# georgeretsi/smirk

Measured on AMD Instinct MI355X. Metric: faces/sec (encode+FLAME+render+generate) @224x224, higher is better.
Workload: dtype f32 results; encoder + generator convs as split-fp16 x3 MFMA with f32 accumulate (fp32-class error), FLAME / raster f32; 1 GPU; BASELINE config 4: full inference incl. SmirkGenerator re-synthesis, 1024-frame batch sharded over the GPUs; global_batch=1024, micro_batch=1024, image=224x224, parallelism=dp1, rccl_ranks_seen=1, collective=none (1 GPU), hw_queues=4

## Files before the change

smirk_amd/csrc/mbconv_image.hip:

```cpp
#include <stdio.h>

#include "common.h"

typedef _Float16 half8 __attribute__((ext_vector_type(8)));

struct MBIArgs {
    const char* x;
    const char* wexp;
    const float *s1, *b1;
    const float* wdw;
    const float *s2, *b2;
    const char* wproj;
    const float *s3, *b3;
    char* out;
    int B, H, W, Cin, mid, Cout, residual, ipw, rows, gsz, nb;
    int off_es, off_wp, off_wc, off_gmap;
    int tile, tiles_x, tiles_y, gpitch;
    int rowsE, nbE, off_gmapE;
};

__device__ __forceinline__ void mbi_barrier() {
    asm volatile("s_waitcnt lgkmcnt(0)" ::: "memory");
    __builtin_amdgcn_s_barrier();
    asm volatile("" ::: "memory");
}

__device__ __forceinline__ int mbi_es(int gi, int c) { return gi * 32 + ((((c >> 2) ^ (gi >> 1)) & 7) << 2) + (c & 3); }

template <int KS, int NT, bool TILE = false, bool PADK = false>
__global__ __launch_bounds__(512, 2) void mbconv_image_kernel(MBIArgs a) {
    extern __shared__ __attribute__((aligned(16))) char mbi_smem[];
    SmirkRangeAccS rng;
    const int strideX = KS * 64 + 16;
    char* Xs = mbi_smem;
    float* Es = (float*)(mbi_smem + a.off_es);
    char* Wp = mbi_smem + a.off_wp;
    float* Wc = (float*)(mbi_smem + a.off_wc);
    short* gmap = (short*)(mbi_smem + a.off_gmap);
    short* gmapE = TILE ? (short*)(mbi_smem + a.off_gmapE) : gmap;
    const int tid = threadIdx.x, lane = tid & 63, wave = tid >> 6, fr = lane & 31, hb = lane >> 5;
    const int ntile = a.tiles_x * a.tiles_y;
    const int tb = TILE ? (int)blockIdx.x / ntile : 0, tt = TILE ? (int)blockIdx.x - tb * ntile : 0;
    const int ty = tt / a.tiles_x, tx = tt - ty * a.tiles_x;
    const int b0 = TILE ? tb : blockIdx.x * a.ipw;
    const int nimg = min(a.ipw, a.B - b0), HW = a.H * a.W, vrows = TILE ? 196 : nimg * HW;
    const int nchunks = (a.mid + 31) / 32;
    const size_t xrow = (size_t)a.Cin * 4;
    const half8 hz = {0, 0, 0, 0, 0, 0, 0, 0};
    const int swave = __builtin_amdgcn_readfirstlane(wave);
    const bool active = swave < a.nb;
    const bool activeE = TILE ? swave < a.nbE : active;
    const int wpbuf = a.Cout * 144;

    half8 we[KS][2];
    float s1v = 0.f, b1v = 0.f;
    auto load_we = [&](int c) {
        int frw = fr;
        asm volatile("" : "+v"(frw));
        const int ch = 32 * c + frw;
        const bool v = ch < a.mid;
        const int chc = min(ch, a.mid - 1);
        const char* wbase = a.wexp;
        asm volatile("" : "+s"(wbase));
        const char* wrow = wbase + (unsigned)chc * (unsigned)(a.Cin * 4);
#pragma unroll
        for (int s = 0; s < KS; ++s) {
            const int g = 2 * s + hb;
            if constexpr (PADK) {
                const int gc = min(g, a.Cin / 8 - 1);
                const half8 t0 = *(const half8*)(wrow + gc * 32), t1h = *(const half8*)(wrow + gc * 32 + 16);
                we[s][0] = g * 8 < a.Cin ? t0 : hz;
                we[s][1] = g * 8 < a.Cin ? t1h : hz;
            } else {
                we[s][0] = *(const half8*)(wrow + g * 32);
                we[s][1] = *(const half8*)(wrow + g * 32 + 16);
            }
        }
        const float t1 = a.s1[chc], t2 = a.b1[chc];
        s1v = v ? t1 : 0.f;
        b1v = v ? t2 : 0.f;
    };
    f32x4 wpv[2];
    float wcv = 0.f;
    auto fetch_stage = [&](int c) {
        int t0 = tid;
        asm volatile("" : "+v"(t0));
#pragma unroll
        for (int u = 0; u < 2; ++u) {
            const int idx = t0 + 512 * u, row = idx >> 3, piece = idx & 7, kg = 4 * c + (piece >> 1);
            const bool ok = row < a.Cout && kg * 8 < a.mid;
            const int rc = min(row, a.Cout - 1), kc = min(kg, a.mid / 8 - 1);
            const f32x4 t = *(const f32x4*)(a.wproj + ((size_t)rc * a.mid + kc * 8) * 4 + (piece & 1) * 16);
            const f32x4 z = {0.f, 0.f, 0.f, 0.f};
            wpv[u] = ok ? t : z;
        }
        {
            const int k = min(t0 >> 5, 10), ch = 32 * c + (t0 & 31), chc = min(ch, a.mid - 1);
            const float* src = k < 9 ? a.wdw + (size_t)k * a.mid : (k == 9 ? a.s2 : a.b2);
            const float t = src[chc];
            wcv = ch < a.mid ? t : 0.f;
        }
    };
    auto store_stage = [&](int c) {
        char* dst = Wp + (c & 1) * wpbuf;
        int t0 = tid;
        asm volatile("" : "+v"(t0));
#pragma unroll
        for (int u = 0; u < 2; ++u) {
            const int idx = t0 + 512 * u, row = idx >> 3, piece = idx & 7;
            if (row < a.Cout) *(f32x4*)(dst + row * 144 + piece * 16) = wpv[u];
        }
        if (t0 < 352) Wc[(c & 1) * 352 + t0] = wcv;
    };

    {
        const int P = a.Cin / 4;
        const char* xb = a.x + (size_t)b0 * HW * xrow;
        const int rowsE = TILE ? 256 : a.rows, total = rowsE * P, vtotal = vrows * P;
        for (int base = 0; base < total; base += 512 * 4) {
            f32x4 xv[4];
#pragma unroll
            for (int u = 0; u < 4; ++u) {
                const int idx = base + 512 * u + tid;
                const f32x4 z = {0.f, 0.f, 0.f, 0.f};
                if (TILE) {
                    const int c = min(idx / P, 255), pc = idx - (idx / P) * P;
                    const int gy = ty * 14 - 1 + (c >> 4), gx = tx * 14 - 1 + (c & 15);
                    const bool ok = idx < total && gy >= 0 && gy < a.H && gx >= 0 && gx < a.W;
                    const int yc = min(max(gy, 0), a.H - 1), xc = min(max(gx, 0), a.W - 1);
                    const f32x4 t = *(const f32x4*)(xb + ((size_t)yc * a.W + xc) * xrow + pc * 16);
                    xv[u] = ok ? t : z;
                } else {
                    const f32x4 t = *(const f32x4*)(xb + (size_t)min(idx, vtotal - 1) * 16);
                    xv[u] = idx < vtotal ? t : z;
                }
            }
#pragma unroll
            for (int u = 0; u < 4; ++u) {
                const int idx = base + 512 * u + tid, row = idx / P, pc = idx - row * P;
                if (idx < total) *(f32x4*)(Xs + row * strideX + pc * 16) = xv[u];
            }
        }
        if (PADK && KS * 4 > P) {
            const int PP = KS * 4 - P;
            for (int idx = tid; idx < rowsE * PP; idx += 512) {
                const int row = idx / PP, pc = P + idx - row * PP;
                *(f32x4*)(Xs + row * strideX + pc * 16) = f32x4{0.f, 0.f, 0.f, 0.f};
            }
        }
        for (int idx = tid; idx < a.gsz * 8; idx += 512) ((f32x4*)Es)[idx] = f32x4{0.f, 0.f, 0.f, 0.f};
        for (int r = tid; r < a.nb * 32; r += 512) {
            int g = -1;
            if (r < vrows) {
                if (TILE) {
                    const int iy = r / 14, ix = r - iy * 14;
                    g = (iy + 1) * 16 + ix + 1;
                } else {
                    const int im = r / HW, rem = r - im * HW, y = rem / a.W, xx = rem - y * a.W;
                    g = (im * (a.H + 2) + y + 1) * (a.W + 2) + xx + 1;
                }
            }
            gmap[r] = (short)g;
        }
        if (TILE)
            for (int r = tid; r < a.nbE * 32; r += 512) {
                const int gy = ty * 14 - 1 + (r >> 4), gx = tx * 14 - 1 + (r & 15);
                const bool ok = r < 256 && gy >= 0 && gy < a.H && gx >= 0 && gx < a.W;
                gmapE[r] = (short)(ok ? r : ~min(r, 255));
            }
    }
    mbi_barrier();

    f32x16 pacc[NT][2];
#pragma unroll
    for (int q = 0; q < NT; ++q)
#pragma unroll
        for (int h = 0; h < 2; ++h)
#pragma unroll
            for (int r = 0; r < 16; ++r) pacc[q][h][r] = 0.f;
    const int myrow = min(wave * 32 + fr, (TILE ? 256 : a.rows) - 1);
    const int mygi = active ? (int)gmap[min(wave * 32 + fr, a.nb * 32 - 1)] : -1;

    auto expand = [&]() {
        if (!activeE) return;
        f32x16 e0, e1;
#pragma unroll
        for (int r = 0; r < 16; ++r) { e0[r] = 0.f; e1[r] = 0.f; }
        const char* arow = Xs + myrow * strideX;
#pragma unroll
        for (int s = 0; s < KS; ++s) {
            const int g = 2 * s + hb;
            const half8 ah = *(const half8*)(arow + g * 32), al = *(const half8*)(arow + g * 32 + 16);
            e0 = __builtin_amdgcn_mfma_f32_32x32x16_f16(ah, we[s][0], e0, 0, 0, 0);
            e1 = __builtin_amdgcn_mfma_f32_32x32x16_f16(ah, we[s][1], e1, 0, 0, 0);
            e1 = __builtin_amdgcn_mfma_f32_32x32x16_f16(al, we[s][0], e1, 0, 0, 0);
            if ((s & 1) || NT == 4) __builtin_amdgcn_sched_barrier(0);
        }
        int rbase = wave * 32 + 4 * hb;
        asm volatile("" : "+v"(rbase));
#pragma unroll
        for (int r = 0; r < 16; ++r) {
            const int gm = gmapE[rbase + (r & 3) + 8 * (r >> 2)];
            const float v = fmaxf((e0[r] + e1[r] * (1.0f / 2048.0f)) * s1v + b1v, 0.f);
            Es[mbi_es(gm >= 0 ? gm : ~gm, fr)] = gm >= 0 ? v : 0.f;
        }
    };


    for (int c = -1; c < nchunks; ++c) {
        const bool more = c + 1 < nchunks;
        if (more) fetch_stage(c + 1);
        half8 dh[2] = {hz, hz}, dl[2] = {hz, hz};
        if (c >= 0 && active && mygi >= 0) {
            const float* wc = Wc + (c & 1) * 352;
#pragma unroll
            for (int s = 0; s < 2; ++s) {
                const int c8 = 8 * (2 * s + hb);
                int gc = mygi;
                asm volatile("" : "+v"(gc));
                float acc[8] = {0.f, 0.f, 0.f, 0.f, 0.f, 0.f, 0.f, 0.f};
#pragma unroll
                for (int ky = 0; ky < 3; ++ky)
#pragma unroll
                    for (int kx = 0; kx < 3; ++kx) {
                        const int gi = gc + (ky - 1) * a.gpitch + (kx - 1);
                        const f32x4 v0 = *(const f32x4*)(Es + mbi_es(gi, c8)), v1 = *(const f32x4*)(Es + mbi_es(gi, c8 + 4));
                        const f32x4 w0 = *(const f32x4*)(wc + (ky * 3 + kx) * 32 + c8), w1 = *(const f32x4*)(wc + (ky * 3 + kx) * 32 + c8 + 4);
#pragma unroll
                        for (int q = 0; q < 4; ++q) { acc[q] = fmaf(v0[q], w0[q], acc[q]); acc[4 + q] = fmaf(v1[q], w1[q], acc[4 + q]); }
                        if (kx == 2 || NT == 4) __builtin_amdgcn_sched_barrier(0);
                    }
                const f32x4 sa = *(const f32x4*)(wc + 9 * 32 + c8), sb = *(const f32x4*)(wc + 9 * 32 + c8 + 4);
                const f32x4 ba = *(const f32x4*)(wc + 10 * 32 + c8), bb = *(const f32x4*)(wc + 10 * 32 + c8 + 4);
#pragma unroll
                for (int q = 0; q < 8; ++q) {
                    const float v = fmaxf(acc[q] * (q < 4 ? sa[q & 3] : sb[q & 3]) + (q < 4 ? ba[q & 3] : bb[q & 3]), 0.f);
                    _Float16 h, l;
                    smirk_split1(v, h, l);
                    dh[s][q] = h; dl[s][q] = l;
                }
            }
        }
        if (more) store_stage(c + 1);
        mbi_barrier();
        if (more) load_we(c + 1);
        if (c >= 0 && active) {
            const char* wp = Wp + (c & 1) * wpbuf;
            int frq = fr;
            asm volatile("" : "+v"(frq));
#pragma unroll
            for (int q = 0; q < NT; ++q) {
                const int co = min(q * 32 + frq, a.Cout - 1);
                const char* brow = wp + co * 144;
#pragma unroll
                for (int s = 0; s < 2; ++s) {
                    const int g = 2 * s + hb;
                    const half8 bhh = *(const half8*)(brow + g * 32), bll = *(const half8*)(brow + g * 32 + 16);
                    pacc[q][0] = __builtin_amdgcn_mfma_f32_32x32x16_f16(dh[s], bhh, pacc[q][0], 0, 0, 0);
                    pacc[q][1] = __builtin_amdgcn_mfma_f32_32x32x16_f16(dh[s], bll, pacc[q][1], 0, 0, 0);
                    pacc[q][1] = __builtin_amdgcn_mfma_f32_32x32x16_f16(dl[s], bhh, pacc[q][1], 0, 0, 0);
                }
                __builtin_amdgcn_sched_barrier(0);
            }
        }
        if (more) expand();
        mbi_barrier();
    }

    if (active) {
        const int lane = __builtin_amdgcn_mbcnt_hi(~0u, __builtin_amdgcn_mbcnt_lo(~0u, 0u)), wave = swave, fr = lane & 31;
        float* tb = Es + wave * (32 * 36);
        char* ob = a.out + (size_t)b0 * HW * a.Cout * 4;
#pragma unroll
        for (int q = 0; q < NT; ++q) {
            if (q * 32 < a.Cout) {
                const int co = q * 32 + fr;
                const float s3 = co < a.Cout ? a.s3[co] : 0.f, b3 = co < a.Cout ? a.b3[co] : 0.f;
#pragma unroll
                for (int r = 0; r < 16; ++r) tb[mfma32_row(r, lane) * 36 + fr] = (pacc[q][0][r] + pacc[q][1][r] * (1.0f / 2048.0f)) * s3 + b3;
                asm volatile("s_waitcnt lgkmcnt(0)" ::: "memory");
#pragma unroll
                for (int it = 0; it < 2; ++it) {
                    const int item = it * 64 + lane, row = item >> 2, g8 = q * 4 + (item & 3);
                    const int r = wave * 32 + row;
                    if (r < vrows && g8 * 8 < a.Cout) {
                        const int iy = r / 14, ix = r - iy * 14;
                        const int xrow_i = TILE ? (iy + 1) * 16 + ix + 1 : r;
                        const size_t opix = TILE ? (size_t)(ty * 14 + iy) * a.W + tx * 14 + ix : (size_t)r;
                        float v[8];
                        *(f32x4*)v = *(const f32x4*)(tb + row * 36 + (item & 3) * 8);
                        *(f32x4*)(v + 4) = *(const f32x4*)(tb + row * 36 + (item & 3) * 8 + 4);
                        if (a.residual) {
                            const char* xr = Xs + xrow_i * strideX + g8 * 32;
                            const half8 hi = *(const half8*)xr, lo = *(const half8*)(xr + 16);
#pragma unroll
                            for (int k = 0; k < 8; ++k) v[k] += (float)hi[k] + (float)lo[k] * (1.0f / 2048.0f);
                        }
                        half8 hi, lo;
                        rng.see8(v);
#pragma unroll
                        for (int k = 0; k < 8; ++k) {
                            _Float16 h, l;
                            smirk_split1(v[k], h, l);
                            hi[k] = h; lo[k] = l;
                        }
                        char* o = ob + (opix * a.Cout + g8 * 8) * 4;
                        *(half8*)o = hi;
                        *(half8*)(o + 16) = lo;
                    }
                }
                asm volatile("s_waitcnt lgkmcnt(0)" ::: "memory");
            }
        }
    }
    rng.commit();
}

struct MbiPlan { int ipw, rows, gsz, nb, off_es, off_wp, off_wc, off_gmap, tile, tiles_x, tiles_y, gpitch, rowsE, nbE, off_gmapE; size_t lds; };
static bool mbi_plan(int H, int W, int Cin, int mid, int Cout, MbiPlan& p) {
    if (H <= 0 || W <= 0 || Cin % 8 || mid % 8 || Cout % 8 || Cin < 16 || Cin > 112 || Cout > 128 || mid <= 0 || Cout <= 0) return false;
    const int KS = (Cin + 15) / 16;
    p.tile = H * W > 224 ? 1 : 0;
    if (p.tile) {
        if (H % 14 || W % 14) return false;
        p.tiles_x = W / 14; p.tiles_y = H / 14; p.gpitch = 16;
        p.ipw = 1; p.rows = 196; p.gsz = 256; p.nb = 7; p.rowsE = 256; p.nbE = 8;
    } else {
        p.tiles_x = p.tiles_y = 1; p.gpitch = W + 2;
        p.ipw = 224 / (H * W);
        if (p.ipw > 8) p.ipw = 8;
        p.rows = p.ipw * H * W;
        p.gsz = p.ipw * (H + 2) * (W + 2);
        p.nb = (p.rows + 31) / 32;
        p.rowsE = p.rows; p.nbE = p.nb;
    }
    if (p.nb > 7 || p.gsz * 128 < p.nb * 32 * 36 * 4) return false;
    size_t o = (size_t)p.rowsE * (KS * 64 + 16);
    o = (o + 15) / 16 * 16; p.off_es = (int)o; o += (size_t)p.gsz * 128;
    p.off_wp = (int)o; o += (size_t)2 * Cout * 144;
    p.off_wc = (int)o; o += 2 * 352 * 4;
    p.off_gmap = (int)o; o += (size_t)p.nb * 32 * 2;
    p.off_gmapE = p.off_gmap;
    if (p.tile) { p.off_gmapE = (int)o; o += (size_t)p.nbE * 32 * 2; }
    p.lds = (o + 15) / 16 * 16;
    return p.lds <= 160 * 1024;
}

static bool mbi_has_variant(int ks, int nt) {
    return (ks == 5 && (nt == 2 || nt == 3 || nt == 4)) || (ks == 6 && (nt == 3 || nt == 4)) || (ks == 7 && (nt == 3 || nt == 4)) ||
           (ks == 4 && (nt == 2 || nt == 3)) || (ks == 2 && nt == 1) || (ks == 3 && nt == 2);
}

extern "C" int smirk_mbconv_image_supported(int H, int W, int Cin, int mid, int Cout, int stride) {
    MbiPlan p;
    if (stride != 1 || !mbi_plan(H, W, Cin, mid, Cout, p)) return 0;
    const int ks = (Cin + 15) / 16, nt = (Cout + 31) / 32;
    if (!mbi_has_variant(ks, nt)) return 0;
    const bool small = (ks == 2 && nt == 1) || (ks == 3 && nt == 2);
    return (small || (!p.tile && Cin % 16 == 0)) ? 1 : 0;
}

template <int KS, int NT, bool TILE = false, bool PADK = false>
static int mbi_launch(const MBIArgs& a, unsigned grid, size_t lds, hipStream_t st) {
    if (const int rc = smirk_raise_dynamic_lds((const void*)mbconv_image_kernel<KS, NT, TILE, PADK>, 160 * 1024)) return rc;
    if (g_smirk_prof_on) {
        char nm[64];
        if (TILE || PADK) snprintf(nm, sizeof(nm), "mbconv_image_kernel<%d,%d,%s,%s>", KS, NT, TILE ? "true" : "false", PADK ? "true" : "false");
        else snprintf(nm, sizeof(nm), "mbconv_image_kernel<%d,%d>", KS, NT);
        const double px = (double)a.B * a.H * a.W;
        smirk_prof_next_mbconv(nm, px, px, a.Cin, a.mid, a.Cout, true, a.residual != 0);
    }
    SMIRK_LAUNCH((mbconv_image_kernel<KS, NT, TILE, PADK>), dim3(grid), dim3(512), lds, st, a);
    return smirk_launch_status();
}

extern "C" int smirk_mbconv_image_split16(const void* x, const void* wexp, const float* s1, const float* b1, const float* wdw, const float* s2,
                                          const float* b2, const void* wproj, const float* s3, const float* b3, int residual, void* out, int B,
                                          int H, int W, int Cin, int mid, int Cout, void* stream) {
    if (!x || !wexp || !s1 || !b1 || !wdw || !s2 || !b2 || !wproj || !s3 || !b3 || !out || B <= 0) return SMIRK_ERR_BAD_ARG;
    if (residual && Cin != Cout) return SMIRK_ERR_BAD_ARG;
    MbiPlan p;
    if (!mbi_plan(H, W, Cin, mid, Cout, p) || !smirk_mbconv_image_supported(H, W, Cin, mid, Cout, 1)) return SMIRK_ERR_UNSUPPORTED;
    MBIArgs a;
    a.x = (const char*)x; a.wexp = (const char*)wexp; a.s1 = s1; a.b1 = b1; a.wdw = wdw; a.s2 = s2; a.b2 = b2; a.wproj = (const char*)wproj;
    a.s3 = s3; a.b3 = b3; a.out = (char*)out; a.B = B; a.H = H; a.W = W; a.Cin = Cin; a.mid = mid; a.Cout = Cout; a.residual = residual;
    a.ipw = p.ipw; a.rows = p.rows; a.gsz = p.gsz; a.nb = p.nb; a.off_es = p.off_es; a.off_wp = p.off_wp; a.off_wc = p.off_wc; a.off_gmap = p.off_gmap;
    a.tile = p.tile; a.tiles_x = p.tiles_x; a.tiles_y = p.tiles_y; a.gpitch = p.gpitch; a.rowsE = p.rowsE; a.nbE = p.nbE; a.off_gmapE = p.off_gmapE;
    const unsigned grid = p.tile ? (unsigned)B * p.tiles_x * p.tiles_y : (unsigned)((B + p.ipw - 1) / p.ipw);
    hipStream_t st = (hipStream_t)stream;
    const int ks = (Cin + 15) / 16, nt = (Cout + 31) / 32;
#define MBI_CASE(K, N) if (ks == K && nt == N) return mbi_launch<K, N>(a, grid, p.lds, st)
    MBI_CASE(5, 3); MBI_CASE(5, 4); MBI_CASE(6, 3); MBI_CASE(7, 4);
    MBI_CASE(4, 2); MBI_CASE(4, 3); MBI_CASE(5, 2); MBI_CASE(6, 4); MBI_CASE(7, 3);
    if (ks == 2 && nt == 1) return p.tile ? mbi_launch<2, 1, true, true>(a, grid, p.lds, st) : mbi_launch<2, 1, false, true>(a, grid, p.lds, st);
    if (ks == 3 && nt == 2) return p.tile ? mbi_launch<3, 2, true, true>(a, grid, p.lds, st) : mbi_launch<3, 2, false, true>(a, grid, p.lds, st);
#undef MBI_CASE
    return SMIRK_ERR_UNSUPPORTED;
}
```

Before: 11390 faces/sec.

## Replace tiled MBConv path with per-wave 2x14 band kernel using 256 threads

The large-image (tiled) path of the fused MBConv kernel is rewritten. Each wave now processes its own 2-row by 14-column output band. Input activations and expand weights are held in registers, and the expanded tile lives in a small per-wave LDS buffer, so the kernel no longer stages a 16x16 haloed tile across 512 threads. Depthwise weights are staged in chunks shared by the four waves. The smaller LDS footprint and 256-thread blocks are meant to raise occupancy and drop the redundant halo expansion of 256 rows per 196 outputs. The trade-off is recomputing the expand for overlapping halo rows across adjacent bands (4 input rows per 2 output rows) and more global weight reloads per chunk.

```diff
diff --git a/smirk_amd/csrc/mbconv_image.hip b/smirk_amd/csrc/mbconv_image.hip
--- a/smirk_amd/csrc/mbconv_image.hip
+++ b/smirk_amd/csrc/mbconv_image.hip
@@ -15,9 +15,11 @@
     char* out;
     int B, H, W, Cin, mid, Cout, residual, ipw, rows, gsz, nb;
     int off_es, off_wp, off_wc, off_gmap;
-    int tile, tiles_x, tiles_y, gpitch;
-    int rowsE, nbE, off_gmapE;
+    int gpitch;
+    int tile, tiles_x, tiles_y, nbands;
 };
+
+extern __shared__ __attribute__((aligned(16))) char mbi_smem[];
 
 __device__ __forceinline__ void mbi_barrier() {
     asm volatile("s_waitcnt lgkmcnt(0)" ::: "memory");
@@ -27,9 +29,8 @@
 
 __device__ __forceinline__ int mbi_es(int gi, int c) { return gi * 32 + ((((c >> 2) ^ (gi >> 1)) & 7) << 2) + (c & 3); }
 
-template <int KS, int NT, bool TILE = false, bool PADK = false>
-__global__ __launch_bounds__(512, 2) void mbconv_image_kernel(MBIArgs a) {
-    extern __shared__ __attribute__((aligned(16))) char mbi_smem[];
+template <int KS, int NT, bool PADK>
+__device__ __forceinline__ void mbi_whole_body(const MBIArgs& a) {
     SmirkRangeAccS rng;
     const int strideX = KS * 64 + 16;
     char* Xs = mbi_smem;
@@ -37,19 +38,14 @@
     char* Wp = mbi_smem + a.off_wp;
     float* Wc = (float*)(mbi_smem + a.off_wc);
     short* gmap = (short*)(mbi_smem + a.off_gmap);
-    short* gmapE = TILE ? (short*)(mbi_smem + a.off_gmapE) : gmap;
     const int tid = threadIdx.x, lane = tid & 63, wave = tid >> 6, fr = lane & 31, hb = lane >> 5;
-    const int ntile = a.tiles_x * a.tiles_y;
-    const int tb = TILE ? (int)blockIdx.x / ntile : 0, tt = TILE ? (int)blockIdx.x - tb * ntile : 0;
-    const int ty = tt / a.tiles_x, tx = tt - ty * a.tiles_x;
-    const int b0 = TILE ? tb : blockIdx.x * a.ipw;
-    const int nimg = min(a.ipw, a.B - b0), HW = a.H * a.W, vrows = TILE ? 196 : nimg * HW;
+    const int b0 = blockIdx.x * a.ipw;
+    const int nimg = min(a.ipw, a.B - b0), HW = a.H * a.W, vrows = nimg * HW;
     const int nchunks = (a.mid + 31) / 32;
     const size_t xrow = (size_t)a.Cin * 4;
     const half8 hz = {0, 0, 0, 0, 0, 0, 0, 0};
     const int swave = __builtin_amdgcn_readfirstlane(wave);
     const bool active = swave < a.nb;
-    const bool activeE = TILE ? swave < a.nbE : active;
     const int wpbuf = a.Cout * 144;
 
     half8 we[KS][2];
@@ -116,24 +112,15 @@
     {
         const int P = a.Cin / 4;
         const char* xb = a.x + (size_t)b0 * HW * xrow;
-        const int rowsE = TILE ? 256 : a.rows, total = rowsE * P, vtotal = vrows * P;
+        const int total = a.rows * P, vtotal = vrows * P;
         for (int base = 0; base < total; base += 512 * 4) {
             f32x4 xv[4];
 #pragma unroll
             for (int u = 0; u < 4; ++u) {
                 const int idx = base + 512 * u + tid;
                 const f32x4 z = {0.f, 0.f, 0.f, 0.f};
-                if (TILE) {
-                    const int c = min(idx / P, 255), pc = idx - (idx / P) * P;
-                    const int gy = ty * 14 - 1 + (c >> 4), gx = tx * 14 - 1 + (c & 15);
-                    const bool ok = idx < total && gy >= 0 && gy < a.H && gx >= 0 && gx < a.W;
-                    const int yc = min(max(gy, 0), a.H - 1), xc = min(max(gx, 0), a.W - 1);
-                    const f32x4 t = *(const f32x4*)(xb + ((size_t)yc * a.W + xc) * xrow + pc * 16);
-                    xv[u] = ok ? t : z;
-                } else {
-                    const f32x4 t = *(const f32x4*)(xb + (size_t)min(idx, vtotal - 1) * 16);
-                    xv[u] = idx < vtotal ? t : z;
-                }
+                const f32x4 t = *(const f32x4*)(xb + (size_t)min(idx, vtotal - 1) * 16);
+                xv[u] = idx < vtotal ? t : z;
             }
 #pragma unroll
             for (int u = 0; u < 4; ++u) {
@@ -143,7 +130,7 @@
         }
         if (PADK && KS * 4 > P) {
             const int PP = KS * 4 - P;
-            for (int idx = tid; idx < rowsE * PP; idx += 512) {
+            for (int idx = tid; idx < a.rows * PP; idx += 512) {
                 const int row = idx / PP, pc = P + idx - row * PP;
                 *(f32x4*)(Xs + row * strideX + pc * 16) = f32x4{0.f, 0.f, 0.f, 0.f};
             }
@@ -152,22 +139,11 @@
         for (int r = tid; r < a.nb * 32; r += 512) {
             int g = -1;
             if (r < vrows) {
-                if (TILE) {
-                    const int iy = r / 14, ix = r - iy * 14;
-                    g = (iy + 1) * 16 + ix + 1;
-                } else {
-                    const int im = r / HW, rem = r - im * HW, y = rem / a.W, xx = rem - y * a.W;
-                    g = (im * (a.H + 2) + y + 1) * (a.W + 2) + xx + 1;
-                }
+                const int im = r / HW, rem = r - im * HW, y = rem / a.W, xx = rem - y * a.W;
+                g = (im * (a.H + 2) + y + 1) * (a.W + 2) + xx + 1;
             }
             gmap[r] = (short)g;
         }
-        if (TILE)
-            for (int r = tid; r < a.nbE * 32; r += 512) {
-                const int gy = ty * 14 - 1 + (r >> 4), gx = tx * 14 - 1 + (r & 15);
-                const bool ok = r < 256 && gy >= 0 && gy < a.H && gx >= 0 && gx < a.W;
-                gmapE[r] = (short)(ok ? r : ~min(r, 255));
-            }
     }
     mbi_barrier();
 
@@ -178,11 +154,11 @@
         for (int h = 0; h < 2; ++h)
 #pragma unroll
             for (int r = 0; r < 16; ++r) pacc[q][h][r] = 0.f;
-    const int myrow = min(wave * 32 + fr, (TILE ? 256 : a.rows) - 1);
+    const int myrow = min(wave * 32 + fr, a.rows - 1);
     const int mygi = active ? (int)gmap[min(wave * 32 + fr, a.nb * 32 - 1)] : -1;
 
     auto expand = [&]() {
-        if (!activeE) return;
+        if (!active) return;
         f32x16 e0, e1;
 #pragma unroll
         for (int r = 0; r < 16; ++r) { e0[r] = 0.f; e1[r] = 0.f; }
@@ -200,7 +176,7 @@
         asm volatile("" : "+v"(rbase));
 #pragma unroll
         for (int r = 0; r < 16; ++r) {
-            const int gm = gmapE[rbase + (r & 3) + 8 * (r >> 2)];
+            const int gm = gmap[rbase + (r & 3) + 8 * (r >> 2)];
             const float v = fmaxf((e0[r] + e1[r] * (1.0f / 2048.0f)) * s1v + b1v, 0.f);
             Es[mbi_es(gm >= 0 ? gm : ~gm, fr)] = gm >= 0 ? v : 0.f;
         }
@@ -284,15 +260,298 @@
                     const int item = it * 64 + lane, row = item >> 2, g8 = q * 4 + (item & 3);
                     const int r = wave * 32 + row;
                     if (r < vrows && g8 * 8 < a.Cout) {
-                        const int iy = r / 14, ix = r - iy * 14;
-                        const int xrow_i = TILE ? (iy + 1) * 16 + ix + 1 : r;
-                        const size_t opix = TILE ? (size_t)(ty * 14 + iy) * a.W + tx * 14 + ix : (size_t)r;
                         float v[8];
                         *(f32x4*)v = *(const f32x4*)(tb + row * 36 + (item & 3) * 8);
                         *(f32x4*)(v + 4) = *(const f32x4*)(tb + row * 36 + (item & 3) * 8 + 4);
                         if (a.residual) {
-                            const char* xr = Xs + xrow_i * strideX + g8 * 32;
+                            const char* xr = Xs + r * strideX + g8 * 32;
                             const half8 hi = *(const half8*)xr, lo = *(const half8*)(xr + 16);
+#pragma unroll
+                            for (int k = 0; k < 8; ++k) v[k] += (float)hi[k] + (float)lo[k] * (1.0f / 2048.0f);
+                        }
+                        half8 hi, lo;
+                        rng.see8(v);
+#pragma unroll
+                        for (int k = 0; k < 8; ++k) {
+                            _Float16 h, l;
+                            smirk_split1(v[k], h, l);
+                            hi[k] = h; lo[k] = l;
+                        }
+                        char* o = ob + ((size_t)r * a.Cout + g8 * 8) * 4;
+                        *(half8*)o = hi;
+                        *(half8*)(o + 16) = lo;
+                    }
+                }
+                asm volatile("s_waitcnt lgkmcnt(0)" ::: "memory");
+            }
+        }
+    }
+    rng.commit();
+}
+
+#define MBB_EB 8192
+#define MBB_STAGE 34
+
+__device__ __forceinline__ void mbb_out_px(int m, int& oy, int& ox) {
+    const int k = m >> 2;
+    oy = (0x96 >> k) & 1;
+    ox = (k >> 1) * 4 + (m & 3);
+}
+
+__device__ __forceinline__ void mbb_fence() { asm volatile("s_waitcnt lgkmcnt(0)" ::: "memory"); }
+
+template <int KS, int NT>
+__device__ __forceinline__ void mbi_band_body(const MBIArgs& a) {
+    SmirkRangeAccS rng;
+    const int tid = threadIdx.x, lane = tid & 63, fr = lane & 31, hb = lane >> 5;
+    const int wave = __builtin_amdgcn_readfirstlane(tid >> 6);
+    float* Wt = (float*)(mbi_smem + 4 * MBB_EB);
+    const int band = (int)blockIdx.x * 4 + wave;
+    const bool has = band < a.nbands;
+    int bid = min(band, a.nbands - 1);
+    const int bx = bid % a.tiles_x; bid /= a.tiles_x;
+    const int by = bid % a.tiles_y;
+    const int b = bid / a.tiles_y;
+    const int oy0 = by * 2, ox0 = bx * 14;
+    const bool interior = oy0 > 0 && oy0 + 2 < a.H && ox0 > 0 && ox0 + 14 < a.W;
+    const unsigned xrow = (unsigned)a.Cin * 4;
+    const int gmax = a.Cin / 8;
+    const int nchunks = (a.mid + 31) / 32;
+    const half8 hz = {0, 0, 0, 0, 0, 0, 0, 0};
+    const char* xb = a.x + (size_t)b * a.H * a.W * xrow;
+
+    auto stage = [&](int c0) {
+        const int total = min(MBB_STAGE, nchunks - c0) * 352;
+        for (int base = 0; base < total; base += 256 * 8) {
+            float cv[8];
+#pragma unroll
+            for (int u = 0; u < 8; ++u) {
+                const int idx = min(base + 256 * u + tid, total - 1), cl = idx / 352, rem = idx - cl * 352, k = rem >> 5;
+                const int ch = 32 * (c0 + cl) + (rem & 31), chc = min(ch, a.mid - 1);
+                const float* src = k < 9 ? a.wdw + (size_t)k * a.mid : (k == 9 ? a.s2 : a.b2);
+                const float t = src[chc];
+                cv[u] = ch < a.mid ? t : 0.f;
+            }
+#pragma unroll
+            for (int u = 0; u < 8; ++u)
+                if (base + 256 * u + tid < total) Wt[base + 256 * u + tid] = cv[u];
+        }
+    };
+    unsigned xo[2], om[2];
+#pragma unroll
+    for (int t = 0; t < 2; ++t) {
+        const int iy = oy0 - 1 + 2 * t + (fr >> 4), ix = ox0 - 1 + (fr & 15);
+        const bool ok = iy >= 0 && iy < a.H && ix >= 0 && ix < a.W;
+        const int yc = min(max(iy, 0), a.H - 1), xc = min(max(ix, 0), a.W - 1);
+        xo[t] = (unsigned)(yc * a.W + xc) * xrow;
+        om[t] = (unsigned)__builtin_amdgcn_ballot_w64(ok) >> (4 * hb);
+    }
+    auto load_x = [&](int t, half8 (*dst)[2]) {
+        const char* px = xb + xo[t];
+#pragma unroll
+        for (int s = 0; s < KS; ++s) {
+            const int g = 2 * s + hb, gc = min(g, gmax - 1);
+            const half8 t0 = *(const half8*)(px + gc * 32), t1 = *(const half8*)(px + gc * 32 + 16);
+            if (s == KS - 1) { dst[s][0] = g < gmax ? t0 : hz; dst[s][1] = g < gmax ? t1 : hz; }
+            else { dst[s][0] = t0; dst[s][1] = t1; }
+        }
+    };
+    half8 xa[2][KS][2];
+    load_x(0, xa[0]);
+    load_x(1, xa[1]);
+    half8 we[KS][2];
+    float s1v, b1v;
+    auto load_we = [&](int c) {
+        const int ch = 32 * c + fr, chc = min(ch, a.mid - 1);
+        const char* wrow = a.wexp + (size_t)chc * xrow;
+#pragma unroll
+        for (int s = 0; s < KS; ++s) {
+            const int g = 2 * s + hb, gc = min(g, gmax - 1);
+            const half8 t0 = *(const half8*)(wrow + gc * 32), t1 = *(const half8*)(wrow + gc * 32 + 16);
+            if (s == KS - 1) { we[s][0] = g < gmax ? t0 : hz; we[s][1] = g < gmax ? t1 : hz; }
+            else { we[s][0] = t0; we[s][1] = t1; }
+        }
+        const float t1 = a.s1[chc], t2 = a.b1[chc];
+        s1v = ch < a.mid ? t1 : 0.f;
+        b1v = ch < a.mid ? t2 : 0.f;
+    };
+    load_we(0);
+    stage(0);
+    mbb_fence();
+    __builtin_amdgcn_s_barrier();
+    asm volatile("" ::: "memory");
+    if (!has) {
+        for (int c0 = MBB_STAGE; c0 < nchunks; c0 += MBB_STAGE) {
+            __builtin_amdgcn_s_barrier();
+            stage(c0);
+            mbb_fence();
+            __builtin_amdgcn_s_barrier();
+        }
+        return;
+    }
+
+    const unsigned ebase = (unsigned)wave * MBB_EB;
+    const unsigned est = ebase + hb * 512 + ((((unsigned)fr >> 2) ^ (hb << 1)) << 4) + (fr & 3) * 4;
+    unsigned ta[9];
+    int my_oy, my_ox;
+    mbb_out_px(fr, my_oy, my_ox);
+#pragma unroll
+    for (int ky = 0; ky < 3; ++ky)
+#pragma unroll
+        for (int kx = 0; kx < 3; ++kx) {
+            const int cell = ((my_oy + ky) * 16 + my_ox + kx) & 63;
+            ta[ky * 3 + kx] = ebase + cell * 128 + ((((cell >> 1) ^ (2 * hb)) & 7) << 4);
+        }
+
+    f32x16 pacc[NT][2];
+#pragma unroll
+    for (int q = 0; q < NT; ++q)
+#pragma unroll
+        for (int h = 0; h < 2; ++h)
+#pragma unroll
+            for (int r = 0; r < 16; ++r) pacc[q][h][r] = 0.f;
+
+    const float* wc = Wt;
+    int crestage = MBB_STAGE;
+    for (int c = 0; c < nchunks; ++c, wc += 352) {
+        if (c == crestage) {
+            mbb_fence();
+            __builtin_amdgcn_s_barrier();
+            stage(c);
+            mbb_fence();
+            __builtin_amdgcn_s_barrier();
+            asm volatile("" ::: "memory");
+            wc = Wt; crestage += MBB_STAGE;
+        }
+#pragma unroll
+        for (int t = 0; t < 2; ++t) {
+            half8 (*cur)[2] = xa[t];
+            unsigned et = est;
+            asm volatile("" : "+v"(et));
+            f32x16 e0, e1;
+#pragma unroll
+            for (int r = 0; r < 16; ++r) { e0[r] = 0.f; e1[r] = 0.f; }
+#pragma unroll
+            for (int s = 0; s < KS; ++s) {
+                e0 = __builtin_amdgcn_mfma_f32_32x32x16_f16(cur[s][0], we[s][0], e0, 0, 0, 0);
+                e1 = __builtin_amdgcn_mfma_f32_32x32x16_f16(cur[s][0], we[s][1], e1, 0, 0, 0);
+                e1 = __builtin_amdgcn_mfma_f32_32x32x16_f16(cur[s][1], we[s][0], e1, 0, 0, 0);
+            }
+            if (interior) {
+#pragma unroll
+                for (int r = 0; r < 16; ++r) {
+                    const int ro = (r & 3) + 8 * (r >> 2);
+                    const unsigned cr = ((r >> 1) & 1) | (((r >> 2) & 1) << 2);
+                    const float v = fmaxf((e0[r] + e1[r] * (1.0f / 2048.0f)) * s1v + b1v, 0.f);
+                    *(float*)(mbi_smem + (et ^ (cr << 4)) + (32 * t + ro) * 128) = v;
+                }
+            } else {
+#pragma unroll
+                for (int r = 0; r < 16; ++r) {
+                    const int ro = (r & 3) + 8 * (r >> 2);
+                    const unsigned cr = ((r >> 1) & 1) | (((r >> 2) & 1) << 2);
+                    const float v = fmaxf((e0[r] + e1[r] * (1.0f / 2048.0f)) * s1v + b1v, 0.f);
+                    *(float*)(mbi_smem + (et ^ (cr << 4)) + (32 * t + ro) * 128) = ((om[t] >> ro) & 1u) ? v : 0.f;
+                }
+            }
+        }
+        if (c + 1 < nchunks) load_we(c + 1);
+        half8 wp[NT][2][2];
+#pragma unroll
+        for (int q = 0; q < NT; ++q) {
+            const int co = q * 32 + fr;
+            const char* wrow = a.wproj + (size_t)(co < a.Cout ? co : 0) * a.mid * 4;
+#pragma unroll
+            for (int s = 0; s < 2; ++s) {
+                const int kg = min(4 * c + 2 * s + hb, a.mid / 8 - 1);
+                const bool v = co < a.Cout && (4 * c + 2 * s + hb) * 8 < a.mid;
+                const half8 t0 = *(const half8*)(wrow + kg * 32), t1 = *(const half8*)(wrow + kg * 32 + 16);
+                wp[q][s][0] = v ? t0 : hz;
+                wp[q][s][1] = v ? t1 : hz;
+            }
+        }
+        mbb_fence();
+        half8 dh[2], dl[2];
+#pragma unroll
+        for (int s = 0; s < 2; ++s) {
+            const int c8 = 8 * (2 * s + hb);
+            float acc[8] = {0.f, 0.f, 0.f, 0.f, 0.f, 0.f, 0.f, 0.f};
+#pragma unroll
+            for (int ky = 0; ky < 3; ++ky)
+#pragma unroll
+                for (int kx = 0; kx < 3; ++kx) {
+                    const int k = ky * 3 + kx;
+                    unsigned tk = ta[k];
+                    asm volatile("" : "+v"(tk));
+                    const f32x4 v0 = *(const f32x4*)(mbi_smem + (tk ^ ((4 * s) << 4))), v1 = *(const f32x4*)(mbi_smem + (tk ^ ((4 * s + 1) << 4)));
+                    const f32x4 w0 = *(const f32x4*)(wc + k * 32 + c8), w1 = *(const f32x4*)(wc + k * 32 + c8 + 4);
+#pragma unroll
+                    for (int q = 0; q < 4; ++q) { acc[q] = fmaf(v0[q], w0[q], acc[q]); acc[4 + q] = fmaf(v1[q], w1[q], acc[4 + q]); }
+                    if (kx == 2 || NT == 1) __builtin_amdgcn_sched_barrier(0);
+                }
+            const f32x4 sa = *(const f32x4*)(wc + 9 * 32 + c8), sb = *(const f32x4*)(wc + 9 * 32 + c8 + 4);
+            const f32x4 ba = *(const f32x4*)(wc + 10 * 32 + c8), bb = *(const f32x4*)(wc + 10 * 32 + c8 + 4);
+#pragma unroll
+            for (int q = 0; q < 8; ++q) {
+                const float v = fmaxf(acc[q] * (q < 4 ? sa[q & 3] : sb[q & 3]) + (q < 4 ? ba[q & 3] : bb[q & 3]), 0.f);
+                _Float16 h, l;
+                smirk_split1(v, h, l);
+                dh[s][q] = h; dl[s][q] = l;
+            }
+        }
+        mbb_fence();
+#pragma unroll
+        for (int q = 0; q < NT; ++q)
+#pragma unroll
+            for (int s = 0; s < 2; ++s) {
+                pacc[q][0] = __builtin_amdgcn_mfma_f32_32x32x16_f16(dh[s], wp[q][s][0], pacc[q][0], 0, 0, 0);
+                pacc[q][1] = __builtin_amdgcn_mfma_f32_32x32x16_f16(dh[s], wp[q][s][1], pacc[q][1], 0, 0, 0);
+                pacc[q][1] = __builtin_amdgcn_mfma_f32_32x32x16_f16(dl[s], wp[q][s][0], pacc[q][1], 0, 0, 0);
+            }
+    }
+
+    {
+        float* tb = (float*)(mbi_smem + ebase);
+        char* ob = a.out + (size_t)b * a.H * a.W * a.Cout * 4;
+        float s3v[NT], b3v[NT];
+        half8 rh[NT][2], rl[NT][2];
+#pragma unroll
+        for (int q = 0; q < NT; ++q) {
+            const int co = q * 32 + fr, coc = min(co, a.Cout - 1);
+            const float t1 = a.s3[coc], t2 = a.b3[coc];
+            s3v[q] = co < a.Cout ? t1 : 0.f;
+            b3v[q] = co < a.Cout ? t2 : 0.f;
+#pragma unroll
+            for (int it = 0; it < 2; ++it) {
+                rh[q][it] = hz; rl[q][it] = hz;
+                if (a.residual) {
+                    const int item = it * 64 + lane, g8 = min(q * 4 + (item & 3), gmax - 1);
+                    int py, px;
+                    mbb_out_px(item >> 2, py, px);
+                    const char* xr = xb + ((size_t)(oy0 + py) * a.W + ox0 + min(px, 13)) * xrow + g8 * 32;
+                    rh[q][it] = *(const half8*)xr; rl[q][it] = *(const half8*)(xr + 16);
+                }
+            }
+        }
+#pragma unroll
+        for (int q = 0; q < NT; ++q) {
+            if (q * 32 < a.Cout) {
+                const float s3 = s3v[q], b3 = b3v[q];
+#pragma unroll
+                for (int r = 0; r < 16; ++r) tb[mfma32_row(r, lane) * 36 + fr] = (pacc[q][0][r] + pacc[q][1][r] * (1.0f / 2048.0f)) * s3 + b3;
+                mbb_fence();
+#pragma unroll
+                for (int it = 0; it < 2; ++it) {
+                    const int item = it * 64 + lane, row = item >> 2, g8 = q * 4 + (item & 3);
+                    int py, px;
+                    mbb_out_px(row, py, px);
+                    if (px < 14 && g8 * 8 < a.Cout) {
+                        const size_t opix = (size_t)(oy0 + py) * a.W + ox0 + px;
+                        float v[8];
+                        *(f32x4*)v = *(const f32x4*)(tb + row * 36 + (item & 3) * 8);
+                        *(f32x4*)(v + 4) = *(const f32x4*)(tb + row * 36 + (item & 3) * 8 + 4);
+                        if (a.residual) {
+                            const half8 hi = rh[q][it], lo = rl[q][it];
 #pragma unroll
                             for (int k = 0; k < 8; ++k) v[k] += (float)hi[k] + (float)lo[k] * (1.0f / 2048.0f);
                         }
@@ -309,39 +568,45 @@
                         *(half8*)(o + 16) = lo;
                     }
                 }
-                asm volatile("s_waitcnt lgkmcnt(0)" ::: "memory");
+                mbb_fence();
             }
         }
     }
     rng.commit();
 }
 
-struct MbiPlan { int ipw, rows, gsz, nb, off_es, off_wp, off_wc, off_gmap, tile, tiles_x, tiles_y, gpitch, rowsE, nbE, off_gmapE; size_t lds; };
+template <int KS, int NT, bool TILE = false, bool PADK = false>
+__global__ __launch_bounds__(TILE ? 256 : 512, TILE && NT == 1 ? 3 : 2) void mbconv_image_kernel(MBIArgs a) {
+    if constexpr (TILE) mbi_band_body<KS, NT>(a);
+    else mbi_whole_body<KS, NT, PADK>(a);
+}
+
+struct MbiPlan { int ipw, rows, gsz, nb, off_es, off_wp, off_wc, off_gmap, tile, tiles_x, tiles_y, gpitch; size_t lds; };
 static bool mbi_plan(int H, int W, int Cin, int mid, int Cout, MbiPlan& p) {
     if (H <= 0 || W <= 0 || Cin % 8 || mid % 8 || Cout % 8 || Cin < 16 || Cin > 112 || Cout > 128 || mid <= 0 || Cout <= 0) return false;
     const int KS = (Cin + 15) / 16;
     p.tile = H * W > 224 ? 1 : 0;
     if (p.tile) {
         if (H % 14 || W % 14) return false;
-        p.tiles_x = W / 14; p.tiles_y = H / 14; p.gpitch = 16;
-        p.ipw = 1; p.rows = 196; p.gsz = 256; p.nb = 7; p.rowsE = 256; p.nbE = 8;
-    } else {
-        p.tiles_x = p.tiles_y = 1; p.gpitch = W + 2;
-        p.ipw = 224 / (H * W);
-        if (p.ipw > 8) p.ipw = 8;
-        p.rows = p.ipw * H * W;
-        p.gsz = p.ipw * (H + 2) * (W + 2);
-        p.nb = (p.rows + 31) / 32;
-        p.rowsE = p.rows; p.nbE = p.nb;
-    }
+        p.tiles_x = W / 14; p.tiles_y = H / 2; p.gpitch = 16;
+        p.ipw = 1; p.rows = 28; p.gsz = 64; p.nb = 1;
+        p.off_es = p.off_wp = p.off_gmap = 0; p.off_wc = 4 * MBB_EB;
+        const int nchunks = (mid + 31) / 32;
+        p.lds = (size_t)4 * MBB_EB + (size_t)(nchunks < MBB_STAGE ? nchunks : MBB_STAGE) * 352 * 4;
+        return true;
+    }
+    p.tiles_x = p.tiles_y = 1; p.gpitch = W + 2;
+    p.ipw = 224 / (H * W);
+    if (p.ipw > 8) p.ipw = 8;
+    p.rows = p.ipw * H * W;
+    p.gsz = p.ipw * (H + 2) * (W + 2);
+    p.nb = (p.rows + 31) / 32;
     if (p.nb > 7 || p.gsz * 128 < p.nb * 32 * 36 * 4) return false;
-    size_t o = (size_t)p.rowsE * (KS * 64 + 16);
+    size_t o = (size_t)p.rows * (KS * 64 + 16);
     o = (o + 15) / 16 * 16; p.off_es = (int)o; o += (size_t)p.gsz * 128;
     p.off_wp = (int)o; o += (size_t)2 * Cout * 144;
     p.off_wc = (int)o; o += 2 * 352 * 4;
     p.off_gmap = (int)o; o += (size_t)p.nb * 32 * 2;
-    p.off_gmapE = p.off_gmap;
-    if (p.tile) { p.off_gmapE = (int)o; o += (size_t)p.nbE * 32 * 2; }
     p.lds = (o + 15) / 16 * 16;
     return p.lds <= 160 * 1024;
 }
@@ -362,7 +627,7 @@
 
 template <int KS, int NT, bool TILE = false, bool PADK = false>
 static int mbi_launch(const MBIArgs& a, unsigned grid, size_t lds, hipStream_t st) {
-    if (const int rc = smirk_raise_dynamic_lds((const void*)mbconv_image_kernel<KS, NT, TILE, PADK>, 160 * 1024)) return rc;
+    if (const int rc = smirk_raise_dynamic_lds((const void*)mbconv_image_kernel<KS, NT, TILE, PADK>, (TILE ? 80 : 160) * 1024)) return rc;
     if (g_smirk_prof_on) {
         char nm[64];
         if (TILE || PADK) snprintf(nm, sizeof(nm), "mbconv_image_kernel<%d,%d,%s,%s>", KS, NT, TILE ? "true" : "false", PADK ? "true" : "false");
@@ -370,7 +635,7 @@
         const double px = (double)a.B * a.H * a.W;
         smirk_prof_next_mbconv(nm, px, px, a.Cin, a.mid, a.Cout, true, a.residual != 0);
     }
-    SMIRK_LAUNCH((mbconv_image_kernel<KS, NT, TILE, PADK>), dim3(grid), dim3(512), lds, st, a);
+    SMIRK_LAUNCH((mbconv_image_kernel<KS, NT, TILE, PADK>), dim3(grid), dim3(TILE ? 256 : 512), lds, st, a);
     return smirk_launch_status();
 }
 
@@ -385,8 +650,11 @@
     a.x = (const char*)x; a.wexp = (const char*)wexp; a.s1 = s1; a.b1 = b1; a.wdw = wdw; a.s2 = s2; a.b2 = b2; a.wproj = (const char*)wproj;
     a.s3 = s3; a.b3 = b3; a.out = (char*)out; a.B = B; a.H = H; a.W = W; a.Cin = Cin; a.mid = mid; a.Cout = Cout; a.residual = residual;
     a.ipw = p.ipw; a.rows = p.rows; a.gsz = p.gsz; a.nb = p.nb; a.off_es = p.off_es; a.off_wp = p.off_wp; a.off_wc = p.off_wc; a.off_gmap = p.off_gmap;
-    a.tile = p.tile; a.tiles_x = p.tiles_x; a.tiles_y = p.tiles_y; a.gpitch = p.gpitch; a.rowsE = p.rowsE; a.nbE = p.nbE; a.off_gmapE = p.off_gmapE;
-    const unsigned grid = p.tile ? (unsigned)B * p.tiles_x * p.tiles_y : (unsigned)((B + p.ipw - 1) / p.ipw);
+    a.tile = p.tile; a.tiles_x = p.tiles_x; a.tiles_y = p.tiles_y; a.gpitch = p.gpitch;
+    const size_t nbands = (size_t)B * p.tiles_x * p.tiles_y;
+    if (p.tile && (nbands > 0x7fffffffu / 4 || (size_t)H * W * Cin * 4 > 0x7fffffffu)) return SMIRK_ERR_UNSUPPORTED;
+    a.nbands = (int)nbands;
+    const unsigned grid = p.tile ? (unsigned)((nbands + 3) / 4) : (unsigned)((B + p.ipw - 1) / p.ipw);
     hipStream_t st = (hipStream_t)stream;
     const int ks = (Cin + 15) / 16, nt = (Cout + 31) / 32;
 #define MBI_CASE(K, N) if (ks == K && nt == N) return mbi_launch<K, N>(a, grid, p.lds, st)
```

New measurement: 11540 faces/sec (median of 6 runs). 1.01x the previous value.
